# PacificBiosciences/trgt

Measured on AMD Instinct MI355X. Metric: loci/s, higher is better.
Workload: dtype u8/u16 (WFA) + f64 (HMM); 1 GPU; BASELINE configs[1]: 10000 synthetic single-motif STR loci per GPU (motif 3-6 bp, allele <= 200 bp), 30 reads/locus HiFi-like, 10% truncated reads (SURVEY.md Appendix E), seed 20250509; contexts_per_gpu=4, loci_per_gpu=10000, reads_per_locus=30, parallelism=loci sharded across 1 GPU(s), no collective

## Files before the change

### trgt_amd/csrc/spans.hip

```cpp
#include <algorithm>
#include <cmath>
#include <optional>

#include "wfa_host.hpp"

namespace trgt {

enum SpanCount : int {
  SC_HEAVY = 0,
  SC_LONG = 1,
  SC_LIGHT = 2,
  SC_ZERO = 3,
  SC_WIN = 4,
  SC_REST = 5,
  SC_KEEP = 6,
  SC_SHORTCUT = 7,
  SC_NOSEED = 8,
  SC_GAPS = 9,
  SC_BAND = 10,
  SC_HREST = 11,
  SC_BANDFAIL = 12,
  SC_LBAND = 13,
  SC_LREST = 14,
  SC_LNOSEED = 15,
  SC_SIBDROP = 16,
  SC_WINCLAIM = 17,
  SC_WINFALL = 18,
  SC_SETDROP = 19,
  SC_FILTER = 20,
  SC_LCSDROP = 21,
  SC_BANDCLAIM = 22,
  SC_BANDFALL = 23,
  SC_BANDREG = 24,
  SC_LBANDCLAIM = 25, SC_LBANDFALL = 26, SC_LBANDREG = 27,
  SC_WORDS = 28
};

struct ScanArgs {
  const uint8_t* flank_blob; const uint8_t* read_blob;
  const uint64_t* piece_off;
  const uint64_t* read_off; const uint32_t* read_len; const uint32_t* read_locus;
  uint64_t n_jobs;
  int32_t flank_len;
  int32_t* pos;
  int32_t* n_match;
  JobDev* wfa_jobs; uint32_t* wfa_count;
  const uint32_t* heavy_len; uint32_t jobs_cap;
  JobDev* wfa_jobs_long; uint32_t long_tlen;
  int32_t min_matches;
  uint8_t* settled;
};

__device__ __forceinline__ uint32_t load_u32(const uint8_t* p) {
  uint32_t v;
  __builtin_memcpy(&v, p, 4);
  return v;
}

__global__ void __launch_bounds__(256) flank_scan_kernel(const ScanArgs a) {
  const uint64_t j = (uint64_t)blockIdx.x * 4 + (threadIdx.x >> 6);
  if (j >= a.n_jobs) return;
  const int lane = threadIdx.x & 63;
  const uint64_t r = j >> 1;
  const int side = (int)(j & 1);
  const int F = a.flank_len, n = (int)a.read_len[r];
  const uint8_t* __restrict__ piece = a.flank_blob + a.piece_off[2 * (uint64_t)a.read_locus[r] + side];
  const uint8_t* __restrict__ read = a.read_blob + a.read_off[r];
  int found = -1;
  if (n >= F) {
    const int last = n - F;
    const uint32_t head = F >= 4 ? load_u32(piece) : 0;
    for (int base = 0; base <= last && found < 0; base += 64) {
      const int p = base + lane;
      bool hit = false;
      if (p <= last) {
        hit = F < 4 || load_u32(read + p) == head;
        if (hit) {
          int i = F >= 4 ? 4 : 0;
          for (; i + 4 <= F; i += 4)
            if (load_u32(read + p + i) != load_u32(piece + i)) { hit = false; break; }
          if (hit)
            for (; i < F; ++i)
              if (read[p + i] != piece[i]) { hit = false; break; }
        }
      }
      const unsigned long long m = __ballot(hit);
      if (m) found = base + (__ffsll((long long)m) - 1);
    }
  }
  if (lane == 0) {
    a.pos[j] = found; a.n_match[j] = -1;
    if (a.settled) a.settled[j] = 0;
    if (found < 0) {
      const bool lng = (uint32_t)n > a.long_tlen;
      const uint32_t slot = atomicAdd(a.wfa_count + (lng ? SC_LONG : SC_HEAVY), 1u);
      JobDev jd;
      jd.pat_off = a.piece_off[2 * (uint64_t)a.read_locus[r] + side]; jd.txt_off = a.read_off[r];
      jd.cigar_off = 0; jd.ops_off = 0; jd.pat_len = (uint32_t)F; jd.txt_len = (uint32_t)n; jd.out_index = (uint32_t)j; jd.pad = 0;
      (lng ? a.wfa_jobs_long : a.wfa_jobs)[slot] = jd;
    }
  }
}

constexpr int WIN_SEGMENTS_DEFAULT = 8;
template <int WIN_SEGMENTS>
__device__ __forceinline__ void piece_window_heads(const uint8_t* __restrict__ read, int n, const uint64_t (&h)[WIN_SEGMENTS], const uint32_t (&h3)[WIN_SEGMENTS], int q, int lane,
                                                   int& kmin_out, int& kmax_out);
template <int WIN_SEGMENTS>
__device__ __forceinline__ void piece_window(const uint8_t* __restrict__ read, int n, const uint8_t* __restrict__ piece, int q, int lane,
                                             int& kmin_out, int& kmax_out) {
  uint64_t h[WIN_SEGMENTS]; uint32_t h3[WIN_SEGMENTS];
#pragma unroll
  for (int i = 0; i < WIN_SEGMENTS; ++i) {
    const uint8_t* __restrict__ seg = piece + i * q;
    h[i] = (uint64_t)load_u32(seg + 4) << 32 | load_u32(seg);
    h3[i] = load_u32(seg + 8);
  }
  piece_window_heads<WIN_SEGMENTS>(read, n, h, h3, q, lane, kmin_out, kmax_out);
}
template <int WIN_SEGMENTS>
__device__ __forceinline__ void piece_window_heads(const uint8_t* __restrict__ read, int n, const uint64_t (&h)[WIN_SEGMENTS], const uint32_t (&h3)[WIN_SEGMENTS], int q, int lane,
                                                   int& kmin_out, int& kmax_out) {
  int kmin = 0x7FFFFFFF, kmax = -0x7FFFFFFF;
  const int last = n - 12;
  for (int base = 0; base <= last; base += 1024) {
    const int off = base + 16 * lane;
    uint32_t w[7] = {0, 0, 0, 0, 0, 0, 0};
    if (off + 28 <= n) {
      uint4 v; uint2 v2; uint32_t v3;
      __builtin_memcpy(&v, read + off, 16); __builtin_memcpy(&v2, read + off + 16, 8); __builtin_memcpy(&v3, read + off + 24, 4);
      w[0] = v.x; w[1] = v.y; w[2] = v.z; w[3] = v.w; w[4] = v2.x; w[5] = v2.y; w[6] = v3;
    } else if (off < n) {
      const int rem = n - off, full = rem >> 2, tail = rem & 3;
#pragma unroll
      for (int k = 0; k < 7; ++k)
        if (k < full) w[k] = load_u32(read + off + 4 * k);
      if (tail && full < 7) {
        const uint32_t t = n >= 4 ? load_u32(read + n - 4) >> (8 * (4 - tail)) : 0u;
        if (n >= 4) {
#pragma unroll
          for (int k = 0; k < 7; ++k) if (k == full) w[k] = t;
        } else {
          for (int b = 4 * full; b < rem; ++b) w[b >> 2] |= (uint32_t)read[off + b] << (8 * (b & 3));
        }
      }
    }
    uint32_t lo[24];
#pragma unroll
    for (int j = 0; j < 24; ++j) {
      const int d = j >> 2, sh = j & 3;
      lo[j] = sh == 0 ? w[d] : __builtin_amdgcn_alignbyte(w[d + 1], w[d], sh);
    }
#pragma unroll
    for (int i = 0; i < WIN_SEGMENTS; ++i) {
      const uint32_t h_lo = (uint32_t)h[i], h_hi = (uint32_t)(h[i] >> 32);
      unsigned long long m[16], any = 0ull;
#pragma unroll
      for (int s16 = 0; s16 < 16; ++s16) { m[s16] = __ballot(lo[s16] == h_lo); any |= m[s16]; }
      if (any == 0ull) continue;
#pragma unroll
      for (int s16 = 0; s16 < 16; ++s16) {
        if (m[s16] != 0ull) {
          asm volatile("" ::: "memory");
          const unsigned long long full = m[s16] & __ballot(lo[s16 + 4] == h_hi && lo[s16 + 8] == h3[i] && off + s16 <= last);
          if (full != 0ull) {
            const int k0 = base + s16 - i * q;
            const int k_lo = k0 + 16 * (int)__builtin_ctzll(full), k_hi = k0 + 16 * (63 - (int)__builtin_clzll(full));
            kmin = k_lo < kmin ? k_lo : kmin; kmax = k_hi > kmax ? k_hi : kmax;
          }
        }
      }
    }
  }
  kmin_out = kmin; kmax_out = kmax;
}

struct WindowArgs {
  const uint8_t* flank_blob; const uint8_t* read_blob;
  const JobDev* wfa_jobs; uint32_t jobs_cap; uint32_t* count;
  JobDev* win_jobs; JobDev* rest_jobs;
  int32_t flank_len, q, margin, spread, tbf;
  int32_t front;
  const JobDev* long_jobs; JobDev* long_rest;
  int32_t hamming_max;
  int32_t indel_ok;
  int32_t* n_match; uint32_t* span4;
  uint8_t* settled;
};
constexpr int WIN_JOBS_PER_WG = 64;
template <int WIN_SEGMENTS>
__global__ void __launch_bounds__(256) flank_window_kernel(const WindowArgs a) {
  __shared__ JobDev l_out[WIN_JOBS_PER_WG];
  __shared__ JobDev l_long[WIN_JOBS_PER_WG];
  __shared__ uint32_t l_nw, l_nr, l_bw, l_br, l_ns, l_ni, l_nl, l_bl;
  const uint32_t n_first = a.count[a.front ? SC_HEAVY : SC_LIGHT], n_light = n_first + (a.long_jobs ? a.count[SC_LONG] : 0u);
  const int lane = threadIdx.x & 63, wave = threadIdx.x >> 6;
  const uint32_t per_wg = min((uint32_t)WIN_JOBS_PER_WG, max(4u, ((n_light + gridDim.x - 1u) / gridDim.x + 3u) & ~3u));
  for (uint32_t c0 = blockIdx.x * per_wg; c0 < n_light; c0 += gridDim.x * per_wg) {
    if (threadIdx.x == 0) { l_nw = 0; l_nr = 0; l_ns = 0; l_ni = 0; l_nl = 0; }
    __syncthreads();
    const uint32_t c1 = c0 + per_wg < n_light ? c0 + per_wg : n_light;
    uint64_t pf_pat = 0, pf_txt = 0, pf_cig = 0, pf_ops = 0;
    uint32_t pf_plen = 0, pf_tlen = 0, pf_oi = 0, pf_pad = 0, pf_hlo[WIN_SEGMENTS], pf_hhi[WIN_SEGMENTS], pf_h3[WIN_SEGMENTS];
#pragma unroll
    for (int sg = 0; sg < WIN_SEGMENTS; ++sg) { pf_hlo[sg] = 0; pf_hhi[sg] = 0; pf_h3[sg] = 0; }
    {
      const uint32_t ij = c0 + (uint32_t)wave + 4u * (uint32_t)lane;
      if (lane < WIN_JOBS_PER_WG / 4 && ij < c1) {
        const JobDev pj = ij >= n_first ? a.long_jobs[ij - n_first] : a.front ? a.wfa_jobs[ij] : a.wfa_jobs[a.jobs_cap - 1u - ij];
        pf_pat = pj.pat_off; pf_txt = pj.txt_off; pf_cig = pj.cigar_off; pf_ops = pj.ops_off; pf_plen = pj.pat_len; pf_tlen = pj.txt_len; pf_oi = pj.out_index; pf_pad = pj.pad;
        if (pj.txt_len >= 12u) {
#pragma unroll
          for (int sg = 0; sg < WIN_SEGMENTS; ++sg) {
            const uint8_t* __restrict__ seg = a.flank_blob + pj.pat_off + sg * a.q;
            pf_hlo[sg] = load_u32(seg); pf_hhi[sg] = load_u32(seg + 4); pf_h3[sg] = load_u32(seg + 8);
          }
        }
      }
    }
    auto lane32 = [](uint32_t v, int j) -> uint32_t { return (uint32_t)__builtin_amdgcn_readlane((int)v, j); };
    auto lane64 = [&](uint64_t v, int j) -> uint64_t { return (uint64_t)lane32((uint32_t)v, j) | ((uint64_t)lane32((uint32_t)(v >> 32), j) << 32); };
    int slot = 0;
    for (uint32_t i = c0 + (uint32_t)wave; i < c1; i += 4, ++slot) {
      const bool is_long = i >= n_first;
      JobDev jd;
      jd.pat_off = lane64(pf_pat, slot); jd.txt_off = lane64(pf_txt, slot); jd.cigar_off = lane64(pf_cig, slot); jd.ops_off = lane64(pf_ops, slot);
      jd.pat_len = lane32(pf_plen, slot); jd.txt_len = lane32(pf_tlen, slot); jd.out_index = lane32(pf_oi, slot); jd.pad = lane32(pf_pad, slot);
      const int n = (int)jd.txt_len, F = a.flank_len;
      int kmin = 1, kmax = 0;
      if (n >= 12) {
        uint64_t h[WIN_SEGMENTS]; uint32_t h3[WIN_SEGMENTS];
#pragma unroll
        for (int sg = 0; sg < WIN_SEGMENTS; ++sg) { h[sg] = (uint64_t)lane32(pf_hlo[sg], slot) | ((uint64_t)lane32(pf_hhi[sg], slot) << 32); h3[sg] = lane32(pf_h3[sg], slot); }
        piece_window_heads<WIN_SEGMENTS>(a.read_blob + jd.txt_off, n, h, h3, a.q, lane, kmin, kmax);
      }
      bool solved = false;
      if (a.hamming_max > 0 && kmin == kmax && kmin >= 0 && kmin + F <= n) {
        const uint8_t* __restrict__ t = a.read_blob + jd.txt_off + kmin;
        const uint8_t* __restrict__ pz = a.flank_blob + jd.pat_off;
        auto differing_bytes = [](uint32_t x) -> uint32_t { return (uint32_t)__builtin_popcount((x | ((x & 0x7F7F7F7Fu) + 0x7F7F7F7Fu)) & 0x80808080u); };
        uint32_t cnt = 0;
        for (int i = lane; i < (F >> 2); i += 64) cnt += differing_bytes(load_u32(t + 4 * i) ^ load_u32(pz + 4 * i));
        if (lane == 63 && (F & 3)) cnt += differing_bytes((load_u32(t + F - 4) ^ load_u32(pz + F - 4)) >> (8 * (4 - (F & 3))));
        const unsigned long long b1 = __ballot(cnt >= 1u);
        uint32_t total = (uint32_t)__popcll(b1);
        if (total <= (uint32_t)a.hamming_max) total += (uint32_t)(__popcll(__ballot(cnt >= 2u)) + __popcll(__ballot(cnt >= 3u)) + __popcll(__ballot(cnt >= 4u)) + __popcll(__ballot(cnt >= 5u)));
        cnt = total;
        if (cnt >= 1u && cnt <= (uint32_t)a.hamming_max) {
          solved = true;
          if (lane == 0) {
            const uint64_t j = jd.out_index;
            a.n_match[j] = F - (int)cnt;
            a.span4[4 * j] = 0u; a.span4[4 * j + 1] = (uint32_t)F; a.span4[4 * j + 2] = (uint32_t)kmin; a.span4[4 * j + 3] = (uint32_t)(kmin + F);
            if (a.settled) a.settled[j] = 1;
            atomicAdd(&l_ns, 1u);
          }
        }
      }
      if (!solved && a.indel_ok && kmax - kmin == 1 && kmin >= 0 && kmax + F <= n && F <= 255) {
        const uint8_t* __restrict__ t = a.read_blob + jd.txt_off + kmin;
        const uint8_t* __restrict__ pz = a.flank_blob + jd.pat_off;
        const int nd = F >> 2, rem = F & 3;
        uint32_t pw = 0, t0 = 0, t1 = 0;
        if (lane < nd) { pw = load_u32(pz + 4 * lane); t0 = load_u32(t + 4 * lane); t1 = load_u32(t + 1 + 4 * lane); }
        else if (lane == nd && rem) { const int sh = 8 * (4 - rem); pw = load_u32(pz + F - 4) >> sh; t0 = load_u32(t + F - 4) >> sh; t1 = load_u32(t + 1 + F - 4) >> sh; }
        auto byte_flags = [](uint32_t x) -> uint32_t { return (x | ((x & 0x7F7F7F7Fu) + 0x7F7F7F7Fu)) & 0x80808080u; };
        const uint32_t m0 = byte_flags(pw ^ t0), m1 = byte_flags(pw ^ t1);
        const unsigned long long b0 = __ballot(m0 != 0u), b1 = __ballot(m1 != 0u);
        auto lcp = [&](unsigned long long b, uint32_t m) -> int {
          if (!b) return F;
          const int l = (int)__builtin_ctzll(b);
          return 4 * l + (__builtin_ctz((uint32_t)__builtin_amdgcn_readlane((int)m, l)) >> 3);
        };
        auto sfx = [&](unsigned long long b, uint32_t m) -> int {
          if (!b) return 0;
          const int l = 63 - (int)__builtin_clzll(b);
          return 4 * l + ((31 - __builtin_clz((uint32_t)__builtin_amdgcn_readlane((int)m, l))) >> 3) + 1;
        };
        auto at_least_4 = [&](unsigned long long b, uint32_t m) -> bool {
          const int lanes = __popcll(b);
          if (lanes >= 4) return true;
          const uint32_t c = (uint32_t)__builtin_popcount(m);
          return lanes + __popcll(__ballot(c >= 2u)) + __popcll(__ballot(c >= 3u)) + __popcll(__ballot(c >= 4u)) >= 4;
        };
        const int lcp0 = lcp(b0, m0), lcp1 = lcp(b1, m1), sfx0 = sfx(b0, m0), sfx1 = sfx(b1, m1);
        const int last_head = (WIN_SEGMENTS - 1) * a.q;
        const bool margins = sfx0 > 13 && sfx1 > 13 && lcp0 < last_head - 1 && lcp1 < last_head - 1;
        const bool ins_ok = sfx1 <= lcp0;
        const bool del_ok = max(sfx0 - 1, 0) <= min(lcp1, F - 1);
        if (margins && ins_ok != del_ok && at_least_4(b0, m0) && at_least_4(b1, m1)) {
          solved = true;
          if (lane == 0) {
            const uint64_t j = jd.out_index;
            const int start = ins_ok ? kmin : kmax, len = ins_ok ? F + 1 : F - 1;
            a.n_match[j] = ins_ok ? F : F - 1;
            a.span4[4 * j] = 0u; a.span4[4 * j + 1] = (uint32_t)F; a.span4[4 * j + 2] = (uint32_t)start; a.span4[4 * j + 3] = (uint32_t)(start + len);
            if (a.settled) a.settled[j] = 1;
            atomicAdd(&l_ns, 1u);
            atomicAdd(&l_ni, 1u);
          }
        }
      }
      if (solved) continue;
      int w0 = 0, wl = 0;
      if (kmin <= kmax && kmax - kmin <= a.spread && (!a.front || (kmin >= 0 && kmax + F <= n))) {
        const int lo = kmin - a.margin;
        w0 = lo > 0 ? lo : 0;
        wl = n - w0 < a.tbf + F ? n - w0 : a.tbf + F;
      }
      if (lane == 0) {
        if (wl > 0) { jd.txt_off += (uint64_t)w0; jd.txt_len = (uint32_t)wl; jd.pad = (uint32_t)w0; l_out[atomicAdd(&l_nw, 1u)] = jd; }
        else if (is_long) l_long[atomicAdd(&l_nl, 1u)] = jd;
        else l_out[WIN_JOBS_PER_WG - 1 - atomicAdd(&l_nr, 1u)] = jd;
      }
    }
    __syncthreads();
    if (threadIdx.x == 0 && l_nw) l_bw = atomicAdd(a.count + SC_WIN, l_nw);
    if (threadIdx.x == 64 && l_nr) l_br = atomicAdd(a.count + (a.front ? SC_NOSEED : SC_REST), l_nr);
    if (threadIdx.x == 65 && l_nl) l_bl = atomicAdd(a.count + SC_LNOSEED, l_nl);
    if (threadIdx.x == 128 && l_ns) atomicAdd(a.count + SC_SHORTCUT, l_ns);
    if (threadIdx.x == 192 && l_ni) atomicAdd(a.count + SC_GAPS, l_ni);
    __syncthreads();
    for (uint32_t i = threadIdx.x; i < l_nw; i += blockDim.x) a.win_jobs[l_bw + i] = l_out[i];
    for (uint32_t i = threadIdx.x; i < l_nr; i += blockDim.x) a.rest_jobs[l_br + i] = l_out[WIN_JOBS_PER_WG - 1 - i];
    for (uint32_t i = threadIdx.x; i < l_nl; i += blockDim.x) a.long_rest[l_bl + i] = l_long[i];
    __syncthreads();
  }
}

constexpr int SCAN_READS_PER_WG = 64;
__global__ void __launch_bounds__(256) flank_scan_wide_kernel(const ScanArgs a) {
  __shared__ JobDev l_jobs[2 * SCAN_READS_PER_WG];
  __shared__ uint32_t l_n, l_n2, l_base, l_base2, l_drop;
  if (threadIdx.x == 0) { l_n = 0; l_n2 = 0; l_drop = 0; }
  __syncthreads();
  const int lane = threadIdx.x & 63;
  const uint64_t n_reads = a.n_jobs >> 1;
  const uint64_t r_begin = (uint64_t)blockIdx.x * SCAN_READS_PER_WG, r_end = r_begin + SCAN_READS_PER_WG < n_reads ? r_begin + SCAN_READS_PER_WG : n_reads;
  const int F = a.flank_len;
  const bool h8 = F >= 8;
  uint32_t pf_n = 0, pf_h0 = 0, pf_h1 = 0, pf_h20 = 0, pf_h21 = 0, pf_heavy = 0;
  uint64_t pf_roff = 0, pf_po0 = 0, pf_po1 = 0;
  {
    const uint64_t rj = r_begin + (threadIdx.x >> 6) + 4ull * (uint64_t)lane;
    if (lane < SCAN_READS_PER_WG / 4 && rj < r_end) {
      pf_n = a.read_len[rj]; pf_roff = a.read_off[rj];
      const uint64_t loc = a.read_locus[rj];
      pf_po0 = a.piece_off[2 * loc]; pf_po1 = a.piece_off[2 * loc + 1];
      if (a.heavy_len) pf_heavy = a.heavy_len[loc];
      if ((int)pf_n >= F) {
        pf_h0 = load_u32(a.flank_blob + pf_po0); pf_h1 = load_u32(a.flank_blob + pf_po1);
        if (h8) { pf_h20 = load_u32(a.flank_blob + pf_po0 + 4); pf_h21 = load_u32(a.flank_blob + pf_po1 + 4); }
      }
    }
  }
  auto from_lane32 = [](uint32_t v, int j) -> uint32_t { return (uint32_t)__builtin_amdgcn_readlane((int)v, j); };
  auto from_lane64 = [&](uint64_t v, int j) -> uint64_t { return (uint64_t)from_lane32((uint32_t)v, j) | ((uint64_t)from_lane32((uint32_t)(v >> 32), j) << 32); };
  int slot = 0;
  for (uint64_t r = r_begin + (threadIdx.x >> 6); r < r_end; r += 4, ++slot) {
  const int n = (int)from_lane32(pf_n, slot);
  const uint64_t po0 = from_lane64(pf_po0, slot), po1 = from_lane64(pf_po1, slot);
  const uint8_t* __restrict__ piece[2] = {a.flank_blob + po0, a.flank_blob + po1};
  const uint64_t r_off = from_lane64(pf_roff, slot);
  const uint32_t heavy_r = from_lane32(pf_heavy, slot);
  const uint8_t* __restrict__ read = a.read_blob + r_off;
  int found[2] = {-1, -1};
  if (n >= F) {
    const int last = n - F;
    const uint32_t head[2] = {from_lane32(pf_h0, slot), from_lane32(pf_h1, slot)};
    const uint32_t head2[2] = {from_lane32(pf_h20, slot), from_lane32(pf_h21, slot)};
    const int nd = F >> 2;
    for (int base = 0; base <= last && (found[0] < 0 || found[1] < 0); base += 1024) {
      const int off = base + 16 * lane;
      uint32_t w[6] = {0, 0, 0, 0, 0, 0};
      if (off + 24 <= n) {
        uint4 q; uint2 q2;
        __builtin_memcpy(&q, read + off, 16); __builtin_memcpy(&q2, read + off + 16, 8);
        w[0] = q.x; w[1] = q.y; w[2] = q.z; w[3] = q.w; w[4] = q2.x; w[5] = q2.y;
      } else if (off <= last) {
        for (int b = 0; b < 24 && off + b < n; ++b) w[b >> 2] |= (uint32_t)read[off + b] << (8 * (b & 3));
      }
      uint32_t m[2] = {0, 0};
      const uint64_t h64[2] = {(uint64_t)head[0] | ((uint64_t)head2[0] << 32), (uint64_t)head[1] | ((uint64_t)head2[1] << 32)};
#pragma unroll
      for (int s16 = 0; s16 < 16; ++s16) {
        const uint32_t win = (s16 & 3) == 0 ? w[s16 >> 2] : __builtin_amdgcn_alignbyte(w[(s16 >> 2) + 1], w[s16 >> 2], s16 & 3);
        if (h8) {
          const uint32_t win2 = (s16 & 3) == 0 ? w[(s16 >> 2) + 1] : __builtin_amdgcn_alignbyte(w[(s16 >> 2) + 2], w[(s16 >> 2) + 1], s16 & 3);
          const uint64_t w64 = (uint64_t)win | ((uint64_t)win2 << 32);
          m[0] |= (uint32_t)(w64 == h64[0]) << s16;
          m[1] |= (uint32_t)(w64 == h64[1]) << s16;
        } else {
          m[0] |= (uint32_t)(win == head[0]) << s16;
          m[1] |= (uint32_t)(win == head[1]) << s16;
        }
      }
      {
        const int room = last - off;
        const uint32_t vmask = room >= 15 ? 0xFFFFu : room < 0 ? 0u : (1u << (room + 1)) - 1u;
        m[0] &= vmask; m[1] &= vmask;
      }
#pragma unroll
      for (int side = 0; side < 2; ++side) {
        if (found[side] >= 0) continue;
        uint32_t mm = m[side];
        for (;;) {
          const unsigned long long lanes = __ballot(mm != 0u);
          if (!lanes) break;
          const int lq = __ffsll((long long)lanes) - 1;
          const uint32_t mq = (uint32_t)__builtin_amdgcn_readlane((int)mm, lq);
          const int sq = __ffs((int)mq) - 1;
          const int p = base + 16 * lq + sq;
          bool ok = true;
          for (int i = lane; i < nd; i += 64) ok = ok && load_u32(read + p + 4 * i) == load_u32(piece[side] + 4 * i);
          if (lane == 63 && (F & 3)) ok = ok && load_u32(read + p + F - 4) == load_u32(piece[side] + F - 4);
          if (__ballot(!ok) == 0ull) { found[side] = p; break; }
          if (lane == lq) mm &= mm - 1u;
        }
      }
    }
  }
  if (lane == 0) {
    for (int side = 0; side < 2; ++side) {
      const uint64_t j = 2 * r + side;
      a.pos[j] = found[side]; a.n_match[j] = -1;
      if (a.settled) a.settled[j] = 0;
      const int room = found[side ^ 1] < 0 ? 0x7FFFFFFF : side ? n - found[0] - F : found[1];
      if (found[side] < 0 && room < a.min_matches) atomicAdd(&l_drop, 1u);
      else if (found[side] < 0) {
        JobDev jd;
        jd.pat_off = side ? po1 : po0; jd.txt_off = r_off;
        jd.cigar_off = 0; jd.ops_off = 0; jd.pat_len = (uint32_t)F; jd.txt_len = (uint32_t)n; jd.out_index = (uint32_t)j; jd.pad = 0;
        if ((uint32_t)n > a.long_tlen) a.wfa_jobs_long[atomicAdd(a.wfa_count + SC_LONG, 1u)] = jd;
        else if (!a.heavy_len || (uint32_t)n < heavy_r) l_jobs[atomicAdd(&l_n, 1u)] = jd;
        else l_jobs[2 * SCAN_READS_PER_WG - 1 - atomicAdd(&l_n2, 1u)] = jd;
      }
    }
  }
  }
  __syncthreads();
  if (threadIdx.x == 0 && l_n) l_base = atomicAdd(a.wfa_count + SC_HEAVY, l_n);
  if (threadIdx.x == 64 && l_n2) l_base2 = atomicAdd(a.wfa_count + SC_LIGHT, l_n2);
  if (threadIdx.x == 128 && l_drop) atomicAdd(a.wfa_count + SC_SIBDROP, l_drop);
  __syncthreads();
  for (uint32_t i = threadIdx.x; i < l_n; i += blockDim.x) a.wfa_jobs[l_base + i] = l_jobs[i];
  for (uint32_t i = threadIdx.x; i < l_n2; i += blockDim.x) a.wfa_jobs[a.jobs_cap - 1u - (l_base2 + i)] = l_jobs[2 * SCAN_READS_PER_WG - 1 - i];
}

constexpr int LCS_MAX_F = 256, LCS_MAX_ADM = 352;
struct SettledArgs {
  const JobDev* jobs; const uint32_t* n_jobs;
  JobDev* out; uint32_t* count;
  const uint8_t* settled; const uint32_t* span4; int32_t min_matches;
  int32_t lcs_max_adm;
  const int32_t* pos; const uint8_t* flank_blob; const uint8_t* read_blob;
};
constexpr int LCS_ROWS = 5;
__device__ __forceinline__ uint32_t lcs_row(uint32_t c) {
  const uint32_t code = (c >> 1) & 3u;
  return ((0x47544341u >> (8u * code)) & 0xFFu) == c ? code : 4u;
}
__device__ __forceinline__ void lcs_step(uint32_t (&V)[8], const uint32_t (*peq)[8][64], uint32_t lane, uint32_t c) {
  const uint32_t row = lcs_row(c);
  uint32_t m[8], carry = 0;
#pragma unroll
  for (int w = 0; w < 8; ++w) m[w] = peq[row][w][lane];
#pragma unroll
  for (int w = 0; w < 8; ++w) {
    const uint32_t u = V[w] & m[w];
    const uint32_t sum = __builtin_addc(V[w], u, carry, &carry);
    V[w] = sum | (V[w] & ~u);
  }
}
__device__ __forceinline__ bool lcs_below(uint32_t (*peq)[8][64], uint32_t lane, const uint8_t* __restrict__ pat, int F, const uint8_t* __restrict__ txt, int n, int min_matches) {
  for (int w = 0; w < 8; ++w) {
    uint32_t x[8];
#pragma unroll
    for (int q = 0; q < 8; ++q) {
      const int b0 = w * 32 + q * 4;
      x[q] = 0;
      if (b0 + 4 <= F) x[q] = load_u32(pat + b0);
      else
        for (int k = 0; b0 + k < F; ++k) x[q] |= (uint32_t)pat[b0 + k] << (8 * k);
    }
    uint32_t m0 = 0, m1 = 0, m2 = 0, m3 = 0;
#pragma unroll
    for (int q = 0; q < 8; ++q)
#pragma unroll
      for (int k = 0; k < 4; ++k) {
        const uint32_t row = lcs_row((x[q] >> (8 * k)) & 0xFFu), sel = (1u << row) | (0u - (row >> 2));
        m0 |= (sel & 1u) << (q * 4 + k); m1 |= ((sel >> 1) & 1u) << (q * 4 + k); m2 |= ((sel >> 2) & 1u) << (q * 4 + k); m3 |= ((sel >> 3) & 1u) << (q * 4 + k);
      }
    const uint32_t valid = F >= (w + 1) * 32 ? 0xFFFFFFFFu : (F > w * 32 ? (1u << (F - w * 32)) - 1u : 0u);
    peq[0][w][lane] = m0 & valid; peq[1][w][lane] = m1 & valid; peq[2][w][lane] = m2 & valid; peq[3][w][lane] = m3 & valid; peq[4][w][lane] = valid;
  }
  uint32_t V[8];
#pragma unroll
  for (int w = 0; w < 8; ++w) V[w] = 0xFFFFFFFFu;
  const int full = n & ~15;
  uint32_t cur[4] = {0, 0, 0, 0}, nxt[4] = {0, 0, 0, 0};
  if (full) {
#pragma unroll
    for (int k = 0; k < 4; ++k) cur[k] = load_u32(txt + 4 * k);
  }
  for (int i = 0; i < full; i += 16) {
    if (i + 16 < full) {
#pragma unroll
      for (int k = 0; k < 4; ++k) nxt[k] = load_u32(txt + i + 16 + 4 * k);
    }
#pragma unroll
    for (int k = 0; k < 4; ++k)
#pragma unroll
      for (int b = 0; b < 4; ++b) lcs_step(V, peq, lane, (cur[k] >> (8 * b)) & 0xFFu);
#pragma unroll
    for (int k = 0; k < 4; ++k) cur[k] = nxt[k];
  }
  for (int i = full; i < n; ++i) lcs_step(V, peq, lane, txt[i]);
  int ones = 0;
#pragma unroll
  for (int w = 0; w < 8; ++w) ones += __popc(V[w]);
  return 256 - ones < min_matches;
}
__global__ void __launch_bounds__(64) settled_sibling_kernel(const SettledArgs a) {
  __shared__ uint32_t l_peq[LCS_ROWS][8][64];
  const uint32_t n = *a.n_jobs, lane = threadIdx.x & 63u;
  for (uint32_t i0 = (blockIdx.x * blockDim.x + threadIdx.x) & ~63u; i0 < n; i0 += gridDim.x * blockDim.x) {
    const uint32_t i = i0 + lane;
    bool stay = false, drop = false, lcs = false;
    JobDev jd;
    if (i < n) {
      jd = a.jobs[i];
      const uint32_t j = jd.out_index, sib = j ^ 1u;
      int room = 0x7FFFFFFF, st = 0, en = 0;
      bool known = false;
      if (a.settled && a.settled[sib]) {
        st = (int)a.span4[4 * (uint64_t)sib + 2]; en = (int)a.span4[4 * (uint64_t)sib + 3]; known = true;
        room = (j & 1u) ? (int)jd.txt_len - en : st;
        drop = room < a.min_matches;
      } else if (a.lcs_max_adm > 0) {
        st = a.pos[sib]; en = st + (int)jd.pat_len; known = st >= 0;
        if (known) room = (j & 1u) ? (int)jd.txt_len - en : st;
      }
      if (known && !drop && a.lcs_max_adm > 0 && jd.pat_len <= (uint32_t)LCS_MAX_F && room >= a.min_matches && room <= a.lcs_max_adm && (uint32_t)room <= jd.txt_len)
        lcs = lcs_below(l_peq, lane, a.flank_blob + jd.pat_off, (int)jd.pat_len, a.read_blob + jd.txt_off + ((j & 1u) ? (uint32_t)en : 0u), room, a.min_matches);
      stay = !drop && !lcs;
    }
    const unsigned long long ms = __ballot(stay), md = __ballot(drop), ml = __ballot(lcs);
    uint32_t base = 0;
    if (lane == 0) {
      if (ms) base = atomicAdd(a.count + SC_FILTER, (uint32_t)__popcll(ms));
      if (md) atomicAdd(a.count + SC_SETDROP, (uint32_t)__popcll(md));
      if (ml) atomicAdd(a.count + SC_LCSDROP, (uint32_t)__popcll(ml));
    }
    base = (uint32_t)__builtin_amdgcn_readfirstlane((int)base);
    if (stay) a.out[base + (uint32_t)__popcll(ms & ((1ull << lane) - 1ull))] = jd;
  }
}

struct WinCheckArgs {
  const JobDev* win_jobs; const uint32_t* n_win; const int32_t* score; uint32_t* span4; int32_t* n_match; int32_t s0;
  JobDev* wfa_jobs; uint32_t* wfa_count; uint32_t jobs_cap; const uint64_t* read_off; const uint32_t* read_len;
  JobDev* long_rest; uint32_t long_tlen;
};
__global__ void window_check_kernel(const WinCheckArgs a) {
  const uint32_t n = *a.n_win;
  for (uint32_t i = blockIdx.x * blockDim.x + threadIdx.x; i < n; i += gridDim.x * blockDim.x) {
    JobDev jd = a.win_jobs[i];
    const uint32_t j = jd.out_index;
    const int32_t sc = a.score[j];
    if (sc != INT32_MIN && -sc <= a.s0 && a.n_match[j] > 0) {
      a.span4[4 * (uint64_t)j + 2] += jd.pad; a.span4[4 * (uint64_t)j + 3] += jd.pad;
    } else {
      a.n_match[j] = -1;
      jd.txt_off = a.read_off[j >> 1]; jd.txt_len = a.read_len[j >> 1]; jd.pad = 0;
      if (a.long_rest && jd.txt_len > a.long_tlen) a.long_rest[atomicAdd(a.wfa_count + SC_LNOSEED, 1u)] = jd;
      else a.wfa_jobs[atomicAdd(a.wfa_count + SC_REST, 1u)] = jd;
    }
  }
}

struct BandArgs {
  const JobDev* keep_jobs; const uint32_t* n_keep; JobDev* band_jobs; JobDev* rest_jobs; uint32_t* count; int32_t s_max;
  const int32_t* score; uint32_t* span4; int32_t* n_match; const uint64_t* read_off; const uint32_t* read_len;
  int32_t i_band, i_rest;
};
__global__ void heavy_band_kernel(const BandArgs a) {
  const uint32_t n = *a.n_keep;
  for (uint32_t i = blockIdx.x * blockDim.x + threadIdx.x; i < n; i += gridDim.x * blockDim.x) {
    JobDev jd = a.keep_jobs[i];
    const uint32_t pad = jd.pad;
    const int s = (int)((pad >> 16) & 0x7FFFu), plen = (int)jd.pat_len, tlen = (int)jd.txt_len, k_end = (int)(pad & 0xFFFFu) - plen;
    const int t0 = max(0, k_end - s), k_hi = min(k_end + s, tlen), t_end = min(tlen, k_end + s + plen);
    if ((pad >> 31) && s <= a.s_max && k_hi >= t0 && t_end > t0) {
      jd.txt_off += (uint64_t)t0; jd.txt_len = (uint32_t)(t_end - t0); jd.pad = (uint32_t)t0;
      jd.ops_off = (uint64_t)(k_hi - t0);
      jd.cigar_off = (uint64_t)s;
      a.band_jobs[atomicAdd(a.count + a.i_band, 1u)] = jd;
    } else {
      jd.pad = 0;
      a.rest_jobs[atomicAdd(a.count + a.i_rest, 1u)] = jd;
    }
  }
}
__global__ void band_check_kernel(const BandArgs a) {
  const uint32_t n = a.count[a.i_band];
  for (uint32_t i = blockIdx.x * blockDim.x + threadIdx.x; i < n; i += gridDim.x * blockDim.x) {
    JobDev jd = a.band_jobs[i];
    const uint32_t j = jd.out_index;
    const int32_t sc = a.score[j];
    if (sc != INT32_MIN && -sc == (int32_t)jd.cigar_off && a.n_match[j] > 0) {
      a.span4[4 * (uint64_t)j + 2] += jd.pad; a.span4[4 * (uint64_t)j + 3] += jd.pad;
    } else {
      a.n_match[j] = -1;
      jd.txt_off = a.read_off[j >> 1]; jd.txt_len = a.read_len[j >> 1]; jd.pad = 0; jd.ops_off = 0; jd.cigar_off = 0;
      a.rest_jobs[atomicAdd(a.count + a.i_rest, 1u)] = jd;
      atomicAdd(a.count + SC_BANDFAIL, 1u);
    }
  }
}

struct CombineArgs {
  uint64_t n_reads; int32_t flank_len; double threshold;
  const int32_t* pos; const int32_t* n_match; const uint32_t* span4;
  int32_t* span_start; int32_t* span_end; uint8_t* lf_hit; uint8_t* rf_hit;
  const uint32_t* count; unsigned long long* cells;
};

__global__ void span_combine_kernel(const CombineArgs a) {
  const uint64_t r = (uint64_t)blockIdx.x * blockDim.x + threadIdx.x;
  if (r == 0 && a.cells) a.cells[2] = a.count[SC_SHORTCUT];
  if (r >= a.n_reads) return;
  int s[2], e[2], hit[2];
  for (int side = 0; side < 2; ++side) {
    const uint64_t j = 2 * r + side;
    s[side] = e[side] = -1; hit[side] = 0;
    if (a.pos[j] >= 0) { s[side] = a.pos[j]; e[side] = a.pos[j] + a.flank_len; hit[side] = 1; }
    else if ((double)(uint64_t)(uint32_t)a.n_match[j] >= a.threshold && a.n_match[j] >= 0) {
      s[side] = (int)a.span4[4 * j + 2]; e[side] = (int)a.span4[4 * j + 3]; hit[side] = 2;
    }
  }
  int ss = -1, ee = -1;
  if (hit[0] && hit[1] && e[0] <= s[1]) { ss = e[0]; ee = s[1]; }
  a.span_start[r] = ss; a.span_end[r] = ee;
  if (a.lf_hit) a.lf_hit[r] = (uint8_t)hit[0];
  if (a.rf_hit) a.rf_hit[r] = (uint8_t)hit[1];
}

__global__ void cells_merge_kernel(unsigned long long* total2, const unsigned long long* heavy) { total2[1] = heavy[0]; total2[0] += heavy[0]; }

struct LongWinArgs {
  const JobDev* jobs; const uint32_t* n_jobs;
  JobDev* sub; uint32_t* parent; uint8_t* sub_keep; uint32_t* n_sub; uint32_t cap;
  uint8_t* job_keep;
  JobDev* kept; uint32_t* n_kept;
  int32_t wl, step;
  const uint32_t* sub_band; uint32_t* job_best; uint32_t* job_rej;
};
__device__ __forceinline__ uint32_t long_windows_of(uint32_t tlen, int wl, int step) {
  return tlen <= (uint32_t)wl ? 1u : (tlen - (uint32_t)wl + (uint32_t)step - 1u) / (uint32_t)step + 1u;
}
__global__ void long_windows_kernel(const LongWinArgs a) {
  const uint32_t n = *a.n_jobs;
  for (uint32_t j = blockIdx.x * blockDim.x + threadIdx.x; j < n; j += gridDim.x * blockDim.x) {
    const JobDev job = a.jobs[j];
    const uint32_t tlen = job.txt_len, nw = long_windows_of(tlen, a.wl, a.step);
    const uint32_t off = atomicAdd(a.n_sub, nw);
    const bool fits = off <= a.cap && nw <= a.cap - off;
    a.job_keep[j] = fits ? 0 : 1;
    if (a.job_best) { a.job_best[j] = 0xFFFFFFFFu; a.job_rej[j] = fits ? 0xFFFFFFFFu : 0u; }
    for (uint32_t w = 0; w < nw && off + w < a.cap; ++w) {
      uint32_t start = fits ? w * (uint32_t)a.step : 0u;
      if (tlen > (uint32_t)a.wl && start + (uint32_t)a.wl > tlen) start = tlen - (uint32_t)a.wl;
      JobDev sj = job;
      sj.txt_off = job.txt_off + start; sj.txt_len = tlen > (uint32_t)a.wl ? (uint32_t)a.wl : tlen; sj.out_index = off + w;
      a.sub[off + w] = sj; a.parent[off + w] = j;
    }
  }
}
__global__ void long_verdict_kernel(const LongWinArgs a) {
  const uint32_t n = min(*a.n_sub, a.cap);
  for (uint32_t s = blockIdx.x * blockDim.x + threadIdx.x; s < n; s += gridDim.x * blockDim.x) {
    const uint32_t p = a.parent[s];
    if (a.sub_keep[s]) a.job_keep[p] = 1;
    if (a.sub_band) {
      const uint32_t b = a.sub_band[s];
      if (b >> 31) {
        const uint64_t kbg = (uint64_t)(b & 0xFFFFu) + (a.sub[s].txt_off - a.jobs[p].txt_off);
        if (kbg < 0x10000u) atomicMin(a.job_best + p, (b & 0x7FFF0000u) | (uint32_t)kbg);
        else atomicMin(a.job_rej + p, 0u);
      } else atomicMin(a.job_rej + p, (b >> 30) ? (b & 0x3FFFFFFFu) : 0u);
    }
  }
}
__global__ void long_kept_kernel(const LongWinArgs a) {
  const uint32_t n = *a.n_jobs;
  for (uint32_t j = blockIdx.x * blockDim.x + threadIdx.x; j < n; j += gridDim.x * blockDim.x)
    if (a.job_keep[j]) {
      JobDev jd = a.jobs[j];
      jd.pad = 0;
      if (a.job_best) {
        const uint32_t best = a.job_best[j];
        if (best != 0xFFFFFFFFu && (best >> 16) < a.job_rej[j]) jd.pad = 0x80000000u | best;
      }
      a.kept[atomicAdd(a.n_kept, 1u)] = jd;
    }
}

struct SpanPlan {
  int64_t min_matches = 0; double threshold = 0; int32_t scan_min_matches = 0;
  int ring_slots = 0; uint32_t long_tlen = 0, short_max = 0, heavy_tlen_max = 0; bool has_long = false;
  int32_t win_m = WIN_SEGMENTS_DEFAULT, win_q = 0, win_s0 = 0, win_margin = 0, win_spread = 0, win_tbf = 0; uint32_t win_tlen = 0;
  int32_t hamming_max = 0, indel_ok = 0; bool win_reg = false;
  bool split = false, use_filter = false, two_streams = false; int64_t flt_tlen = 0;
  bool heavy_window = false;
  bool settled_rule = false;
  int32_t lcs_max_adm = 0;
  bool sibling_pass = false;
  bool heavy_band = false;
  bool band_reg = false;
  bool long_window = false;
  bool long_filter = false, long_band = false; int64_t long_wl = 0, long_step = 0; uint64_t long_cap = 0;
  int flank_threads = 0, heavy_threads = 0, win_threads = 0, band_threads = 0, band_s_max = 0; bool early_reject = false, count_offsets = false;
};
static SpanPlan span_plan(const trgt_hip_ctx* c, const trgt_span_params& p, uint64_t n_jobs, uint32_t max_read_len, uint32_t heavy_tlen_max, bool have_heavy_len, bool span_only) {
// ... 454 lines not shown
```

Before: 5.293 million loci/s.

## Software-pipeline read window loads across rounds and jobs in seed scan kernels

Both the window kernel and the scan kernel now issue the global loads for the next 1024-byte round, or the next job's first round, before processing the current one, so load latency overlaps the compare and ballot work. Out-of-range lanes read from a spare in-bounds pointer instead of branching. The flank pattern word is loaded once per job and reused in the Hamming and indel checks, and the second-stage ballot loop is grouped by four shifts to skip empty groups. This adds register pressure and an extra speculative load per job, and the prefetch state can go stale if the early-exit and have flags are handled incorrectly.

```diff
diff --git a/trgt_amd/csrc/spans.hip b/trgt_amd/csrc/spans.hip
--- a/trgt_amd/csrc/spans.hip
+++ b/trgt_amd/csrc/spans.hip
@@ -103,47 +103,37 @@
 }
 
 constexpr int WIN_SEGMENTS_DEFAULT = 8;
+struct WindowRound { uint32_t d0, d1, d2, d3, d4, d5, d6; };
+__device__ __forceinline__ WindowRound window_round_request(const uint8_t* __restrict__ read, int n, int base, const uint8_t* __restrict__ spare, int lane) {
+  const int off = base + 16 * lane;
+  const uint8_t* __restrict__ p = off + 28 <= n ? read + off : spare;
+  typedef uint32_t dwords4 __attribute__((ext_vector_type(4), aligned(1)));
+  typedef uint32_t dwords3 __attribute__((ext_vector_type(3), aligned(1)));
+  const dwords4 v = *reinterpret_cast<const dwords4*>(p);
+  const dwords3 v2 = *reinterpret_cast<const dwords3*>(p + 16);
+  return WindowRound{v.x, v.y, v.z, v.w, v2.x, v2.y, v2.z};
+}
 template <int WIN_SEGMENTS>
 __device__ __forceinline__ void piece_window_heads(const uint8_t* __restrict__ read, int n, const uint64_t (&h)[WIN_SEGMENTS], const uint32_t (&h3)[WIN_SEGMENTS], int q, int lane,
-                                                   int& kmin_out, int& kmax_out);
-template <int WIN_SEGMENTS>
-__device__ __forceinline__ void piece_window(const uint8_t* __restrict__ read, int n, const uint8_t* __restrict__ piece, int q, int lane,
-                                             int& kmin_out, int& kmax_out) {
-  uint64_t h[WIN_SEGMENTS]; uint32_t h3[WIN_SEGMENTS];
-#pragma unroll
-  for (int i = 0; i < WIN_SEGMENTS; ++i) {
-    const uint8_t* __restrict__ seg = piece + i * q;
-    h[i] = (uint64_t)load_u32(seg + 4) << 32 | load_u32(seg);
-    h3[i] = load_u32(seg + 8);
-  }
-  piece_window_heads<WIN_SEGMENTS>(read, n, h, h3, q, lane, kmin_out, kmax_out);
-}
-template <int WIN_SEGMENTS>
-__device__ __forceinline__ void piece_window_heads(const uint8_t* __restrict__ read, int n, const uint64_t (&h)[WIN_SEGMENTS], const uint32_t (&h3)[WIN_SEGMENTS], int q, int lane,
-                                                   int& kmin_out, int& kmax_out) {
+                                                   int& kmin_out, int& kmax_out, WindowRound& wn, bool have, const uint8_t* __restrict__ next_read, int next_n,
+                                                   const uint8_t* __restrict__ spare) {
   int kmin = 0x7FFFFFFF, kmax = -0x7FFFFFFF;
   const int last = n - 12;
+  const int nn = next_n >= 12 ? next_n : 0;
+  WindowRound cur = have ? wn : window_round_request(read, n, 0, spare, lane);
   for (int base = 0; base <= last; base += 1024) {
     const int off = base + 16 * lane;
-    uint32_t w[7] = {0, 0, 0, 0, 0, 0, 0};
-    if (off + 28 <= n) {
-      uint4 v; uint2 v2; uint32_t v3;
-      __builtin_memcpy(&v, read + off, 16); __builtin_memcpy(&v2, read + off + 16, 8); __builtin_memcpy(&v3, read + off + 24, 4);
-      w[0] = v.x; w[1] = v.y; w[2] = v.z; w[3] = v.w; w[4] = v2.x; w[5] = v2.y; w[6] = v3;
-    } else if (off < n) {
+    const bool more = base + 1024 <= last;
+    wn = window_round_request(more ? read : next_read, more ? n : nn, more ? base + 1024 : 0, spare, lane);
+    const bool own = off + 28 <= n;
+    uint32_t w[7] = {own ? cur.d0 : 0u, own ? cur.d1 : 0u, own ? cur.d2 : 0u, own ? cur.d3 : 0u, own ? cur.d4 : 0u, own ? cur.d5 : 0u, own ? cur.d6 : 0u};
+    if (off + 28 > n && off < n) {
       const int rem = n - off, full = rem >> 2, tail = rem & 3;
-#pragma unroll
-      for (int k = 0; k < 7; ++k)
-        if (k < full) w[k] = load_u32(read + off + 4 * k);
-      if (tail && full < 7) {
-        const uint32_t t = n >= 4 ? load_u32(read + n - 4) >> (8 * (4 - tail)) : 0u;
-        if (n >= 4) {
-#pragma unroll
-          for (int k = 0; k < 7; ++k) if (k == full) w[k] = t;
-        } else {
-          for (int b = 4 * full; b < rem; ++b) w[b >> 2] |= (uint32_t)read[off + b] << (8 * (b & 3));
-        }
-      }
+      uint32_t g[7];
+#pragma unroll
+      for (int k = 0; k < 7; ++k) g[k] = load_u32(read + (off + 4 * k < n - 4 ? off + 4 * k : n - 4));
+#pragma unroll
+      for (int k = 0; k < 7; ++k) w[k] = k < full ? g[k] : k == full && tail ? g[k] >> (8 * (4 - tail)) : 0u;
     }
     uint32_t lo[24];
 #pragma unroll
@@ -159,18 +149,25 @@
       for (int s16 = 0; s16 < 16; ++s16) { m[s16] = __ballot(lo[s16] == h_lo); any |= m[s16]; }
       if (any == 0ull) continue;
 #pragma unroll
-      for (int s16 = 0; s16 < 16; ++s16) {
-        if (m[s16] != 0ull) {
+      for (int g = 0; g < 4; ++g) {
+        if ((m[4 * g] | m[4 * g + 1] | m[4 * g + 2] | m[4 * g + 3]) != 0ull) {
           asm volatile("" ::: "memory");
-          const unsigned long long full = m[s16] & __ballot(lo[s16 + 4] == h_hi && lo[s16 + 8] == h3[i] && off + s16 <= last);
-          if (full != 0ull) {
-            const int k0 = base + s16 - i * q;
-            const int k_lo = k0 + 16 * (int)__builtin_ctzll(full), k_hi = k0 + 16 * (63 - (int)__builtin_clzll(full));
-            kmin = k_lo < kmin ? k_lo : kmin; kmax = k_hi > kmax ? k_hi : kmax;
+#pragma unroll
+          for (int s16 = 4 * g; s16 < 4 * g + 4; ++s16) {
+            if (m[s16] != 0ull) {
+              asm volatile("" ::: "memory");
+              const unsigned long long full = m[s16] & __ballot(lo[s16 + 4] == h_hi && lo[s16 + 8] == h3[i] && off + s16 <= last);
+              if (full != 0ull) {
+                const int k0 = base + s16 - i * q;
+                const int k_lo = k0 + 16 * (int)__builtin_ctzll(full), k_hi = k0 + 16 * (63 - (int)__builtin_clzll(full));
+                kmin = k_lo < kmin ? k_lo : kmin; kmax = k_hi > kmax ? k_hi : kmax;
+              }
+            }
           }
         }
       }
     }
+    cur = wn;
   }
   kmin_out = kmin; kmax_out = kmax;
 }
@@ -220,6 +217,8 @@
     }
     auto lane32 = [](uint32_t v, int j) -> uint32_t { return (uint32_t)__builtin_amdgcn_readlane((int)v, j); };
     auto lane64 = [&](uint64_t v, int j) -> uint64_t { return (uint64_t)lane32((uint32_t)v, j) | ((uint64_t)lane32((uint32_t)(v >> 32), j) << 32); };
+    WindowRound wn = {0, 0, 0, 0, 0, 0, 0};
+    bool have = false;
     int slot = 0;
     for (uint32_t i = c0 + (uint32_t)wave; i < c1; i += 4, ++slot) {
       const bool is_long = i >= n_first;
@@ -227,21 +226,32 @@
       jd.pat_off = lane64(pf_pat, slot); jd.txt_off = lane64(pf_txt, slot); jd.cigar_off = lane64(pf_cig, slot); jd.ops_off = lane64(pf_ops, slot);
       jd.pat_len = lane32(pf_plen, slot); jd.txt_len = lane32(pf_tlen, slot); jd.out_index = lane32(pf_oi, slot); jd.pad = lane32(pf_pad, slot);
       const int n = (int)jd.txt_len, F = a.flank_len;
+      const bool next_job = i + 4u < c1;
+      const int next_n = next_job ? (int)lane32(pf_tlen, next_job ? slot + 1 : slot) : 0;
+      const uint64_t next_txt = lane64(pf_txt, next_job ? slot + 1 : slot);
+      const uint8_t* __restrict__ pz = a.flank_blob + jd.pat_off;
+      const int pz_nd = F >> 2;
+      uint32_t pz_w = 0;
+      if (n >= 12 && a.hamming_max > 0 && F >= 4) {
+        if (lane < pz_nd) pz_w = load_u32(pz + 4 * lane);
+        else if ((F & 3) && (lane == pz_nd || lane == 63)) pz_w = load_u32(pz + F - 4);
+      }
       int kmin = 1, kmax = 0;
       if (n >= 12) {
         uint64_t h[WIN_SEGMENTS]; uint32_t h3[WIN_SEGMENTS];
 #pragma unroll
         for (int sg = 0; sg < WIN_SEGMENTS; ++sg) { h[sg] = (uint64_t)lane32(pf_hlo[sg], slot) | ((uint64_t)lane32(pf_hhi[sg], slot) << 32); h3[sg] = lane32(pf_h3[sg], slot); }
-        piece_window_heads<WIN_SEGMENTS>(a.read_blob + jd.txt_off, n, h, h3, a.q, lane, kmin, kmax);
-      }
+        piece_window_heads<WIN_SEGMENTS>(a.read_blob + jd.txt_off, n, h, h3, a.q, lane, kmin, kmax, wn, have, a.read_blob + next_txt, next_n, pz);
+        have = next_n >= 12;
+      } else have = false;
       bool solved = false;
       if (a.hamming_max > 0 && kmin == kmax && kmin >= 0 && kmin + F <= n) {
         const uint8_t* __restrict__ t = a.read_blob + jd.txt_off + kmin;
-        const uint8_t* __restrict__ pz = a.flank_blob + jd.pat_off;
         auto differing_bytes = [](uint32_t x) -> uint32_t { return (uint32_t)__builtin_popcount((x | ((x & 0x7F7F7F7Fu) + 0x7F7F7F7Fu)) & 0x80808080u); };
         uint32_t cnt = 0;
-        for (int i = lane; i < (F >> 2); i += 64) cnt += differing_bytes(load_u32(t + 4 * i) ^ load_u32(pz + 4 * i));
-        if (lane == 63 && (F & 3)) cnt += differing_bytes((load_u32(t + F - 4) ^ load_u32(pz + F - 4)) >> (8 * (4 - (F & 3))));
+        if (lane < (F >> 2)) cnt = differing_bytes(load_u32(t + 4 * lane) ^ pz_w);
+        for (int i = lane + 64; i < (F >> 2); i += 64) cnt += differing_bytes(load_u32(t + 4 * i) ^ load_u32(pz + 4 * i));
+        if (lane == 63 && (F & 3)) cnt += differing_bytes((load_u32(t + F - 4) ^ (pz_nd <= 63 ? pz_w : load_u32(pz + F - 4))) >> (8 * (4 - (F & 3))));
         const unsigned long long b1 = __ballot(cnt >= 1u);
         uint32_t total = (uint32_t)__popcll(b1);
         if (total <= (uint32_t)a.hamming_max) total += (uint32_t)(__popcll(__ballot(cnt >= 2u)) + __popcll(__ballot(cnt >= 3u)) + __popcll(__ballot(cnt >= 4u)) + __popcll(__ballot(cnt >= 5u)));
@@ -259,11 +269,10 @@
       }
       if (!solved && a.indel_ok && kmax - kmin == 1 && kmin >= 0 && kmax + F <= n && F <= 255) {
         const uint8_t* __restrict__ t = a.read_blob + jd.txt_off + kmin;
-        const uint8_t* __restrict__ pz = a.flank_blob + jd.pat_off;
         const int nd = F >> 2, rem = F & 3;
         uint32_t pw = 0, t0 = 0, t1 = 0;
-        if (lane < nd) { pw = load_u32(pz + 4 * lane); t0 = load_u32(t + 4 * lane); t1 = load_u32(t + 1 + 4 * lane); }
-        else if (lane == nd && rem) { const int sh = 8 * (4 - rem); pw = load_u32(pz + F - 4) >> sh; t0 = load_u32(t + F - 4) >> sh; t1 = load_u32(t + 1 + F - 4) >> sh; }
+        if (lane < nd) { pw = pz_w; t0 = load_u32(t + 4 * lane); t1 = load_u32(t + 1 + 4 * lane); }
+        else if (lane == nd && rem) { const int sh = 8 * (4 - rem); pw = pz_w >> sh; t0 = load_u32(t + F - 4) >> sh; t1 = load_u32(t + 1 + F - 4) >> sh; }
         auto byte_flags = [](uint32_t x) -> uint32_t { return (x | ((x & 0x7F7F7F7Fu) + 0x7F7F7F7Fu)) & 0x80808080u; };
         const uint32_t m0 = byte_flags(pw ^ t0), m1 = byte_flags(pw ^ t1);
         const unsigned long long b0 = __ballot(m0 != 0u), b1 = __ballot(m1 != 0u);
@@ -356,9 +365,25 @@
   }
   auto from_lane32 = [](uint32_t v, int j) -> uint32_t { return (uint32_t)__builtin_amdgcn_readlane((int)v, j); };
   auto from_lane64 = [&](uint64_t v, int j) -> uint64_t { return (uint64_t)from_lane32((uint32_t)v, j) | ((uint64_t)from_lane32((uint32_t)(v >> 32), j) << 32); };
+  struct ScanRound { uint32_t d0, d1, d2, d3, d4, d5; };
+  auto round_request = [&](const uint8_t* __restrict__ rd, int rn, int base, const uint8_t* __restrict__ spare) -> ScanRound {
+    typedef uint32_t dwords4 __attribute__((ext_vector_type(4), aligned(1)));
+    typedef uint32_t dwords2 __attribute__((ext_vector_type(2), aligned(1)));
+    const int off = base + 16 * lane;
+    const uint8_t* __restrict__ p = off + 24 <= rn ? rd + off : spare;
+    const dwords4 q = *reinterpret_cast<const dwords4*>(p);
+    const dwords2 q2 = *reinterpret_cast<const dwords2*>(p + 16);
+    return ScanRound{q.x, q.y, q.z, q.w, q2.x, q2.y};
+  };
+  ScanRound wn = {0, 0, 0, 0, 0, 0};
+  bool have = false;
   int slot = 0;
   for (uint64_t r = r_begin + (threadIdx.x >> 6); r < r_end; r += 4, ++slot) {
   const int n = (int)from_lane32(pf_n, slot);
+  const bool next_read = r + 4 < r_end;
+  const int next_n = next_read ? (int)from_lane32(pf_n, next_read ? slot + 1 : slot) : 0;
+  const uint64_t next_off = from_lane64(pf_roff, next_read ? slot + 1 : slot);
+  bool have_next = false;
   const uint64_t po0 = from_lane64(pf_po0, slot), po1 = from_lane64(pf_po1, slot);
   const uint8_t* __restrict__ piece[2] = {a.flank_blob + po0, a.flank_blob + po1};
   const uint64_t r_off = from_lane64(pf_roff, slot);
@@ -370,14 +395,18 @@
     const uint32_t head[2] = {from_lane32(pf_h0, slot), from_lane32(pf_h1, slot)};
     const uint32_t head2[2] = {from_lane32(pf_h20, slot), from_lane32(pf_h21, slot)};
     const int nd = F >> 2;
+    const uint8_t* __restrict__ spare = n >= 24 ? read : reinterpret_cast<const uint8_t*>(a.wfa_count);
+    static_assert(SC_WORDS * 4 >= 24, "the counter block holds a lane's 24 spare bytes");
+    ScanRound cur = have ? wn : round_request(read, n, 0, spare);
     for (int base = 0; base <= last && (found[0] < 0 || found[1] < 0); base += 1024) {
       const int off = base + 16 * lane;
-      uint32_t w[6] = {0, 0, 0, 0, 0, 0};
-      if (off + 24 <= n) {
-        uint4 q; uint2 q2;
-        __builtin_memcpy(&q, read + off, 16); __builtin_memcpy(&q2, read + off + 16, 8);
-        w[0] = q.x; w[1] = q.y; w[2] = q.z; w[3] = q.w; w[4] = q2.x; w[5] = q2.y;
-      } else if (off <= last) {
+      const bool more = base + 1024 <= last;
+      have_next = !more && next_n >= F;
+      wn = round_request(more ? read : a.read_blob + next_off, more ? n : have_next ? next_n : 0, more ? base + 1024 : 0, spare);
+      const bool own = off + 24 <= n;
+      uint32_t w[6] = {own ? cur.d0 : 0u, own ? cur.d1 : 0u, own ? cur.d2 : 0u, own ? cur.d3 : 0u, own ? cur.d4 : 0u, own ? cur.d5 : 0u};
+      cur = wn;
+      if (off + 24 > n && off <= last) {
         for (int b = 0; b < 24 && off + b < n; ++b) w[b >> 2] |= (uint32_t)read[off + b] << (8 * (b & 3));
       }
       uint32_t m[2] = {0, 0};
@@ -420,6 +449,7 @@
       }
     }
   }
+  have = have_next;
   if (lane == 0) {
     for (int side = 0; side < 2; ++side) {
       const uint64_t j = 2 * r + side;
```

Result: slower. 5.162 million loci/s (-2.5%).
